# jiazhihao/ROC

Hardware: AMD Instinct MI355X
Metric: per-epoch training time (s), 2-layer GCN on Reddit (lower is better)
Workload: dtype bf16; 1 GPU; model=gcn-2layer-608-256-64, graph=reddit-synthetic-232965n-114848857e, global_batch=232965, parallelism=graph-partition x1 (single-gpu)

## Files before the change

### roc_amd/csrc/bindings.cpp

```cpp
#include <torch/extension.h>

void spmm(torch::Tensor out, torch::Tensor x, torch::Tensor rowptr,
          torch::Tensor colidx, c10::optional<torch::Tensor> deg_dst,
          c10::optional<torch::Tensor> deg_src,
          c10::optional<torch::Tensor> row_order, bool accumulate,
          int64_t col_base, int64_t ncols);
void rowscale(torch::Tensor out, torch::Tensor x, torch::Tensor scale);
void cast_rowscale(torch::Tensor out, torch::Tensor x,
                   c10::optional<torch::Tensor> scale);
void relu_fwd(torch::Tensor out, torch::Tensor x);
void sigmoid_fwd(torch::Tensor out, torch::Tensor x);
void relu_bwd(torch::Tensor dx, torch::Tensor dy, torch::Tensor y);
void sigmoid_bwd(torch::Tensor dx, torch::Tensor dy, torch::Tensor y);
void ewise_add(torch::Tensor out, torch::Tensor a, torch::Tensor b);
void ewise_mul(torch::Tensor out, torch::Tensor a, torch::Tensor b);
void dropout_fwd(torch::Tensor out, torch::Tensor x, double p, int64_t seed,
                 int64_t offset, c10::optional<torch::Tensor> counter);
void softmax_ce(torch::Tensor dl, torch::Tensor metrics, torch::Tensor logits,
                torch::Tensor labels, torch::Tensor mask, double grad_scale,
                int64_t num_classes);
void adam_step(torch::Tensor w, torch::Tensor g, torch::Tensor m,
               torch::Tensor v, double alpha, double b1, double b2, double eps,
               double wd, c10::optional<torch::Tensor> step,
               double decay_rate, int64_t decay_steps);
void gemm_rr(torch::Tensor C, torch::Tensor A, torch::Tensor Bt, bool relu,
             c10::optional<torch::Tensor> row_scale);
void gemm_atb(torch::Tensor C, torch::Tensor A, torch::Tensor B);
void spmm_refresh_knobs();
void spmm_edge(torch::Tensor out, torch::Tensor x, torch::Tensor rowptr,
               torch::Tensor colidx, torch::Tensor edge_val,
               c10::optional<torch::Tensor> deg_dst,
               c10::optional<torch::Tensor> row_order, bool accumulate);
void edge_dot(torch::Tensor dw, torch::Tensor dy, torch::Tensor x,
              torch::Tensor rowptr, torch::Tensor colidx);
void edge_softmax_fwd(torch::Tensor alpha, torch::Tensor s,
                      torch::Tensor rowptr);
void edge_softmax_bwd(torch::Tensor ds, torch::Tensor dalpha,
                      torch::Tensor alpha, torch::Tensor rowptr);
void att_softmax_fwd(torch::Tensor alpha, torch::Tensor s_src,
                     torch::Tensor s_dst, torch::Tensor rowptr,
                     torch::Tensor colidx, double slope);
void att_softmax_bwd(torch::Tensor dsrc, torch::Tensor dsdst,
                     torch::Tensor dalpha, torch::Tensor alpha,
                     torch::Tensor s_src, torch::Tensor s_dst,
                     torch::Tensor rowptr, torch::Tensor colidx,
                     double slope);
void register_graph_cpu(pybind11::module_& m);

PYBIND11_MODULE(TORCH_EXTENSION_NAME, m) {
  m.doc() = "roc_amd hand-written CDNA4 (gfx950) kernels";
  m.def("spmm", &spmm, "CSR SpMM neighbor aggregation (fused deg-norm)",
        pybind11::arg("out"), pybind11::arg("x"), pybind11::arg("rowptr"),
        pybind11::arg("colidx"), pybind11::arg("deg_dst") = pybind11::none(),
        pybind11::arg("deg_src") = pybind11::none(),
        pybind11::arg("row_order") = pybind11::none(),
        pybind11::arg("accumulate") = false,
        pybind11::arg("col_base") = 0, pybind11::arg("ncols") = 0);
  m.def("rowscale", &rowscale);
  m.def("cast_rowscale", &cast_rowscale,
        "fp32 -> bf16 cast with optional row scale (strip epilogue)",
        pybind11::arg("out"), pybind11::arg("x"),
        pybind11::arg("scale") = pybind11::none());
  m.def("relu_fwd", &relu_fwd);
  m.def("sigmoid_fwd", &sigmoid_fwd);
  m.def("relu_bwd", &relu_bwd);
  m.def("sigmoid_bwd", &sigmoid_bwd);
  m.def("ewise_add", &ewise_add);
  m.def("ewise_mul", &ewise_mul);
  m.def("dropout_fwd", &dropout_fwd, pybind11::arg("out"), pybind11::arg("x"),
        pybind11::arg("p"), pybind11::arg("seed"), pybind11::arg("offset"),
        pybind11::arg("counter") = pybind11::none());
  m.def("softmax_ce", &softmax_ce, pybind11::arg("dl"), pybind11::arg("metrics"),
        pybind11::arg("logits"), pybind11::arg("labels"), pybind11::arg("mask"),
        pybind11::arg("grad_scale"), pybind11::arg("num_classes") = -1);
  m.def("adam_step", &adam_step, pybind11::arg("w"), pybind11::arg("g"),
        pybind11::arg("m"), pybind11::arg("v"), pybind11::arg("alpha"),
        pybind11::arg("b1"), pybind11::arg("b2"), pybind11::arg("eps"),
        pybind11::arg("wd"), pybind11::arg("step") = pybind11::none(),
        pybind11::arg("decay_rate") = 1.0,
        pybind11::arg("decay_steps") = 100);
  m.def("gemm_rr", &gemm_rr, "C = A @ Bt^T (bf16 MFMA, fused relu/rowscale)",
        pybind11::arg("C"), pybind11::arg("A"), pybind11::arg("Bt"),
        pybind11::arg("relu"), pybind11::arg("row_scale") = pybind11::none());
  m.def("gemm_atb", &gemm_atb, "C += A^T @ B (fp32 split-K accumulate)");
  m.def("spmm_refresh_knobs", &spmm_refresh_knobs,
        "re-read ROC_SPMM_* env knobs (A/B harness only)");
  m.def("spmm_edge", &spmm_edge,
        "per-edge-weighted CSR SpMM (edge-tensor consumer)",
        pybind11::arg("out"), pybind11::arg("x"), pybind11::arg("rowptr"),
        pybind11::arg("colidx"), pybind11::arg("edge_val"),
        pybind11::arg("deg_dst") = pybind11::none(),
        pybind11::arg("row_order") = pybind11::none(),
        pybind11::arg("accumulate") = false);
  m.def("edge_dot", &edge_dot,
        "dw[e] = <dy[row_e], x[col_e]> (edge-value gradient)");
  m.def("edge_softmax_fwd", &edge_softmax_fwd,
        "per-row segment softmax over edge scores (GAT attention)");
  m.def("edge_softmax_bwd", &edge_softmax_bwd);
  m.def("att_softmax_fwd", &att_softmax_fwd,
        "fused GAT attention: lrelu(s_src[col]+s_dst[row]) -> softmax");
  m.def("att_softmax_bwd", &att_softmax_bwd);
  register_graph_cpu(m);
}
```

### roc_amd/csrc/spmm.hip

```cpp

#include "row_team.h"

namespace {

template <typename T>
struct RawVec { using type = float4; };
template <>
struct RawVec<unsigned short> { using type = uint4; };

__device__ __forceinline__ uint4 load_raw(const unsigned short* p) {
  return *reinterpret_cast<const uint4*>(p);
}
__device__ __forceinline__ float4 load_raw(const float* p) {
  return *reinterpret_cast<const float4*>(p);
}
__device__ __forceinline__ void acc_add(float* acc, const uint4& r, float w) {
  acc[0] += w * bf16_lo(r.x); acc[1] += w * bf16_hi(r.x);
  acc[2] += w * bf16_lo(r.y); acc[3] += w * bf16_hi(r.y);
  acc[4] += w * bf16_lo(r.z); acc[5] += w * bf16_hi(r.z);
  acc[6] += w * bf16_lo(r.w); acc[7] += w * bf16_hi(r.w);
}
__device__ __forceinline__ void acc_add(float* acc, const float4& r, float w) {
  acc[0] += w * r.x; acc[1] += w * r.y; acc[2] += w * r.z; acc[3] += w * r.w;
}

typedef __attribute__((ext_vector_type(4))) float f32x4v;

template <typename T>
struct GlobalGather {
  const T* x;
  int64_t D;
  int64_t col0;
  __device__ __forceinline__ typename RawVec<T>::type load(int u) const {
    return load_raw(x + (int64_t)u * D + col0);
  }
};

template <typename T>
struct BufferGather {
  __amdgpu_buffer_rsrc_t rsrc;
  unsigned dbytes;
  unsigned colbytes;
  __device__ __forceinline__ typename RawVec<T>::type load(int u) const {
    const f32x4v v = __builtin_amdgcn_raw_buffer_load_b128(
        rsrc, (unsigned)u * dbytes + colbytes, 0, 0);
    return __builtin_bit_cast(typename RawVec<T>::type, v);
  }
};

template <int N, typename T, typename LD, typename USE>
__device__ __forceinline__ void gather_group(
    const LD& ld, const int* __restrict__ colidx, int64_t e, USE&& use) {
  int u[N];
  typename RawVec<T>::type r[N];
#pragma unroll
  for (int i = 0; i < N; ++i) u[i] = colidx[e + i];
#pragma unroll
  for (int i = 0; i < N; ++i) r[i] = ld.load(u[i]);
#pragma unroll
  for (int i = 0; i < N; ++i) use(i, u[i], r[i]);
}

enum class Weight { kNone, kSrc, kEdge };

template <int N, typename T, Weight W, typename LD>
__device__ __forceinline__ void accum_group(
    float* __restrict__ acc, const LD& ld, const int* __restrict__ colidx,
    const float* __restrict__ weight, int64_t e) {
  float w[N];
  if constexpr (W == Weight::kEdge) {
#pragma unroll
    for (int i = 0; i < N; ++i) w[i] = weight[e + i];
  }
  gather_group<N, T>(ld, colidx, e,
                     [&](int i, int u, const typename RawVec<T>::type& r) {
    if constexpr (W == Weight::kEdge) acc_add(acc, r, w[i]);
    else if constexpr (W == Weight::kSrc) acc_add(acc, r, weight[u]);
    else acc_add(acc, r, 1.f);
  });
}

template <typename T, int UN, Weight W, typename LD>
__device__ __forceinline__ void row_accum_vec(
    float* __restrict__ acc, const LD& ld, const int* __restrict__ colidx,
    const float* __restrict__ weight, int64_t e, int64_t e1) {
  if constexpr (UN >= 16)
    for (; e + 15 < e1; e += 16) accum_group<16, T, W>(acc, ld, colidx, weight, e);
  if constexpr (UN >= 8)
    for (; e + 7 < e1; e += 8) accum_group<8, T, W>(acc, ld, colidx, weight, e);
  for (; e + 3 < e1; e += 4) accum_group<4, T, W>(acc, ld, colidx, weight, e);
  for (; e < e1; ++e) accum_group<1, T, W>(acc, ld, colidx, weight, e);
}

template <typename T, Weight W>
__device__ void row_accum_tail(
    float* __restrict__ acc, const T* __restrict__ x, int64_t ld, int64_t col0,
    int nvalid, const int* __restrict__ colidx,
    const float* __restrict__ weight, int64_t e0, int64_t e1) {
  for (int64_t e = e0; e < e1; ++e) {
    const int u0 = colidx[e];
    const T* r = x + (int64_t)u0 * ld + col0;
    const float w0 =
        W == Weight::kEdge ? weight[e] : (weight ? weight[u0] : 1.f);
    for (int j = 0; j < nvalid; ++j) acc[j] += w0 * elt_to_f32(r[j]);
  }
}

template <typename T, typename OT, int TEAM, int UN, bool BUF, Weight W>
__global__ __launch_bounds__(kBlock) void spmm_kernel(
    OT* __restrict__ out, const T* __restrict__ x,
    const int64_t* __restrict__ rowptr, const int* __restrict__ colidx,
    const float* __restrict__ deg_dst, const float* __restrict__ weight,
    const int* __restrict__ row_order, int num_rows, int64_t ld,
    int64_t col_base, int64_t col_end, bool accumulate, unsigned x_bytes) {
  constexpr int EPU = EltTraits<T>::kPerVec;
  const RowTeam<TEAM> rt;

  const int64_t col0 =
      col_base + ((int64_t)blockIdx.y * TEAM + rt.lane) * EPU;
  const bool full = (col0 + EPU) <= col_end;
  const int nvalid =
      full ? EPU : (col0 < col_end ? (int)(col_end - col0) : 0);

  if (full) {
    for (int ri = rt.team; ri < num_rows; ri += rt.nteams) {
      const int row = row_order ? row_order[ri] : ri;
      const int64_t e0 = rowptr[row];
      const int64_t e1 = rowptr[row + 1];
      float acc[EPU];
      OT* o = out + (int64_t)row * ld + col0;
      if (accumulate) {
#pragma unroll
        for (int j = 0; j < EPU; ++j) acc[j] = elt_to_f32(o[j]);
      } else {
#pragma unroll
        for (int j = 0; j < EPU; ++j) acc[j] = 0.f;
      }
      if constexpr (BUF) {
        BufferGather<T> g{
            __builtin_amdgcn_make_buffer_rsrc((void*)x, (short)0, x_bytes,
                                              0x00020000),
            (unsigned)(ld * sizeof(T)), (unsigned)(col0 * sizeof(T))};
        row_accum_vec<T, UN, W>(acc, g, colidx, weight, e0, e1);
      } else {
        GlobalGather<T> g{x, ld, col0};
        row_accum_vec<T, UN, W>(acc, g, colidx, weight, e0, e1);
      }
      if (deg_dst) {
        const float s = deg_dst[row];
#pragma unroll
        for (int j = 0; j < EPU; ++j) acc[j] *= s;
      }
      store_vec(o, acc);
    }
  } else if (nvalid > 0) {
    for (int ri = rt.team; ri < num_rows; ri += rt.nteams) {
      const int row = row_order ? row_order[ri] : ri;
      float acc[EPU];
      OT* o = out + (int64_t)row * ld + col0;
      for (int j = 0; j < nvalid; ++j)
        acc[j] = accumulate ? elt_to_f32(o[j]) : 0.f;
      row_accum_tail<T, W>(acc, x, ld, col0, nvalid, colidx, weight,
                           rowptr[row], rowptr[row + 1]);
      const float s = deg_dst ? deg_dst[row] : 1.f;
      for (int j = 0; j < nvalid; ++j) f32_to_elt(acc[j] * s, o + j);
    }
  }
}

struct SpmmKnobs {
  int team_override;
  int unroll;
  bool allow_buffer;
};

static SpmmKnobs read_spmm_knobs() {
  SpmmKnobs k{0, 16, true};
  if (const char* e = getenv("ROC_SPMM_TEAM")) {
    const int t = atoi(e);
    if (t == 8 || t == 16 || t == 32 || t == 64) k.team_override = t;
  }
  if (const char* e = getenv("ROC_SPMM_UNROLL")) k.unroll = atoi(e);
  if (const char* e = getenv("ROC_SPMM_BUFFER")) k.allow_buffer = e[0] != '0';
  return k;
}

static SpmmKnobs g_spmm_knobs;
static bool g_spmm_knobs_read = false;

static const SpmmKnobs& spmm_knobs() {
  if (!g_spmm_knobs_read) {
    g_spmm_knobs = read_spmm_knobs();
    g_spmm_knobs_read = true;
  }
  return g_spmm_knobs;
}

template <typename T, typename OT, int UN, Weight W>
void launch_spmm(OT* out, const T* x, const int64_t* rowptr,
                 const int* colidx, const float* deg_dst, const float* weight,
                 const int* row_order, int num_rows, int64_t ld,
                 int64_t col_base, int64_t col_end, bool accumulate,
                 size_t x_elems, int team_override, hipStream_t stream) {
  constexpr int EPU = EltTraits<T>::kPerVec;
  const int64_t units = (col_end - col_base + EPU - 1) / EPU;
  const int team = team_override ? team_override : row_team_size(units);
  const dim3 grid =
      row_team_grid(num_rows, team, (int)((units + team - 1) / team));
  const size_t xb = x_elems * sizeof(T);
  const bool buf = xb < (size_t)UINT_MAX && spmm_knobs().allow_buffer;
  const unsigned x_bytes = (unsigned)(buf ? xb : 0);
  if (team < 16) row_order = nullptr;
  dispatch_team(team, [&](auto team_c) {
    dispatch_bool(buf, [&](auto buf_c) {
      hipLaunchKernelGGL(
          (spmm_kernel<T, OT, decltype(team_c)::value, UN,
                       decltype(buf_c)::value, W>),
          grid, dim3(kBlock), 0, stream, out, x, rowptr, colidx, deg_dst,
          weight, row_order, num_rows, ld, col_base, col_end, accumulate,
          x_bytes);
    });
  });
}

template <typename T, int EPU>
__device__ __forceinline__ float dot_unit(
    const float (&a)[EPU], const typename RawVec<T>::type& r) {
  float b[EPU];
#pragma unroll
  for (int j = 0; j < EPU; ++j) b[j] = 0.f;
  acc_add(b, r, 1.f);
  float p = 0.f;
#pragma unroll
  for (int j = 0; j < EPU; ++j) p += a[j] * b[j];
  return p;
}

template <int N, typename T, int TEAM, int EPU>
__device__ __forceinline__ void edge_dot_group(
    float* __restrict__ dw, const float (&a)[EPU], const GlobalGather<T>& g,
    const int* __restrict__ colidx, int64_t e, bool live, int lane) {
  float p[N];
#pragma unroll
  for (int i = 0; i < N; ++i) p[i] = 0.f;
  if (live)
    gather_group<N, T>(g, colidx, e,
                       [&](int i, int, const typename RawVec<T>::type& r) {
      p[i] = dot_unit<T>(a, r);
    });
#pragma unroll
  for (int i = 0; i < N; ++i) p[i] = team_reduce_sum<TEAM>(p[i]);
  if (lane == 0) {
#pragma unroll
    for (int i = 0; i < N; ++i) dw[e + i] = p[i];
  }
}

template <typename T, int TEAM>
__global__ __launch_bounds__(kBlock) void edge_dot_kernel(
    float* __restrict__ dw, const T* __restrict__ dy,
    const T* __restrict__ x, const int64_t* __restrict__ rowptr,
    const int* __restrict__ colidx, int num_rows, int64_t D) {
  constexpr int EPU = EltTraits<T>::kPerVec;
  using Raw = typename RawVec<T>::type;
  const RowTeam<TEAM> rt;
  const int lane = rt.lane;
  if ((int64_t)TEAM * EPU >= D && D % EPU == 0) {
    const bool live = lane < (int)(D / EPU);
    const GlobalGather<T> g{x, D, (int64_t)lane * EPU};
    for (int row = rt.team; row < num_rows; row += rt.nteams) {
      const int64_t e0 = rowptr[row], e1 = rowptr[row + 1];
      float a[EPU] = {0.f};
      if (live) acc_add(a, load_raw(dy + (int64_t)row * D + g.col0), 1.f);
      int64_t e = e0;
      for (; e + 3 < e1; e += 4)
        edge_dot_group<4, T, TEAM>(dw, a, g, colidx, e, live, lane);
      for (; e < e1; ++e)
        edge_dot_group<1, T, TEAM>(dw, a, g, colidx, e, live, lane);
    }
    return;
  }
  for (int row = rt.team; row < num_rows; row += rt.nteams) {
    const int64_t e0 = rowptr[row], e1 = rowptr[row + 1];
    const T* dyr = dy + (int64_t)row * D;
    for (int64_t e = e0; e < e1; ++e) {
      const T* xr = x + (int64_t)colidx[e] * D;
      float p = 0.f;
      for (int64_t c = (int64_t)lane * EPU; c + EPU <= D;
           c += (int64_t)TEAM * EPU) {
        const Raw a = load_raw(dyr + c);
        const Raw b = load_raw(xr + c);
        float ta[EPU] = {0.f}, tb[EPU] = {0.f};
        acc_add(ta, a, 1.f);
        acc_add(tb, b, 1.f);
#pragma unroll
        for (int j = 0; j < EPU; ++j) p += ta[j] * tb[j];
      }
      for (int64_t j = (D / EPU) * EPU + lane; j < D; j += TEAM)
        p += elt_to_f32(dyr[j]) * elt_to_f32(xr[j]);
      p = team_reduce_sum<TEAM>(p);
      if (lane == 0) dw[e] = p;
    }
  }
}

template <typename T>
void launch_edge_dot(float* dw, const T* dy, const T* x,
                     const int64_t* rowptr, const int* colidx, int num_rows,
                     int64_t D, hipStream_t stream) {
  constexpr int EPU = EltTraits<T>::kPerVec;
  const int team = row_team_size((D + EPU - 1) / EPU);
  dispatch_team(team, [&](auto team_c) {
    hipLaunchKernelGGL((edge_dot_kernel<T, decltype(team_c)::value>),
                       row_team_grid(num_rows, team), dim3(kBlock), 0, stream,
                       dw, dy, x, rowptr, colidx, num_rows, D);
  });
}

void check_csr(const torch::Tensor& rowptr, const torch::Tensor& colidx,
               int num_rows) {
  ROC_CHECK_DEV_CONT(rowptr);
  ROC_CHECK_DEV_CONT(colidx);
  TORCH_CHECK(rowptr.scalar_type() == torch::kInt64, "rowptr must be int64");
  TORCH_CHECK(colidx.scalar_type() == torch::kInt32, "colidx must be int32");
  TORCH_CHECK(rowptr.size(0) == num_rows + 1, "rowptr size mismatch");
}

template <typename T>
const T* opt_ptr(const c10::optional<torch::Tensor>& t) {
  return t.has_value() ? t->data_ptr<T>() : nullptr;
}

}

void spmm_refresh_knobs() { g_spmm_knobs_read = false; }

void spmm(torch::Tensor out, torch::Tensor x, torch::Tensor rowptr,
          torch::Tensor colidx, c10::optional<torch::Tensor> deg_dst,
          c10::optional<torch::Tensor> deg_src,
          c10::optional<torch::Tensor> row_order, bool accumulate,
          int64_t col_base, int64_t ncols) {
  ROC_CHECK_DEV_CONT(out);
  ROC_CHECK_DEV_CONT(x);
  TORCH_CHECK(out.scalar_type() == x.scalar_type() ||
                  (out.scalar_type() == torch::kFloat32 &&
                   x.scalar_type() == torch::kBFloat16),
              "dtype mismatch (out must match x, or be fp32 for bf16 x)");
  const int num_rows = (int)out.size(0);
  const int64_t D = out.size(1);
  TORCH_CHECK(x.size(1) == D, "feature dim mismatch");
  check_csr(rowptr, colidx, num_rows);
  const int64_t col_end = ncols > 0 ? col_base + ncols : D;
  TORCH_CHECK(col_base >= 0 && col_base < col_end && col_end <= D,
              "bad column window");
  const float* ds = opt_ptr<float>(deg_src);
  const SpmmKnobs& kn = spmm_knobs();
  auto stream = roc_stream();
  dispatch_elt(x.scalar_type(), "spmm", [&](auto xt) {
    dispatch_elt(out.scalar_type(), "spmm", [&](auto ot) {
      using T = typename decltype(xt)::type;
      using OT = typename decltype(ot)::type;
      if constexpr (sizeof(OT) >= sizeof(T)) {
        auto go = [&](auto un_c, auto w_c) {
          launch_spmm<T, OT, decltype(un_c)::value, decltype(w_c)::value>(
              (OT*)out.data_ptr(), (const T*)x.data_ptr(),
              rowptr.data_ptr<int64_t>(), colidx.data_ptr<int>(),
              opt_ptr<float>(deg_dst), ds, opt_ptr<int>(row_order), num_rows,
              D, col_base, col_end, accumulate, (size_t)x.numel(),
              kn.team_override, stream);
        };
        auto by_weight = [&](auto un_c) {
          if (ds) go(un_c, std::integral_constant<Weight, Weight::kSrc>{});
          else go(un_c, std::integral_constant<Weight, Weight::kNone>{});
        };
        if (kn.unroll >= 16) by_weight(std::integral_constant<int, 16>{});
        else if (kn.unroll >= 8) by_weight(std::integral_constant<int, 8>{});
        else by_weight(std::integral_constant<int, 4>{});
      }
    });
  });
  ROC_HIP_CHECK(hipGetLastError());
}

void spmm_edge(torch::Tensor out, torch::Tensor x, torch::Tensor rowptr,
               torch::Tensor colidx, torch::Tensor edge_val,
               c10::optional<torch::Tensor> deg_dst,
               c10::optional<torch::Tensor> row_order, bool accumulate) {
  ROC_CHECK_DEV_CONT(out);
  ROC_CHECK_DEV_CONT(x);
  ROC_CHECK_DEV_CONT(edge_val);
  TORCH_CHECK(edge_val.scalar_type() == torch::kFloat32,
              "edge_val must be fp32");
  TORCH_CHECK(edge_val.numel() == colidx.numel(), "edge_val size mismatch");
  TORCH_CHECK(out.scalar_type() == x.scalar_type(), "dtype mismatch");
  const int num_rows = (int)out.size(0);
  const int64_t D = out.size(1);
  TORCH_CHECK(x.size(1) == D, "feature dim mismatch");
  check_csr(rowptr, colidx, num_rows);
  auto stream = roc_stream();
  dispatch_elt(x.scalar_type(), "spmm_edge", [&](auto xt) {
    using T = typename decltype(xt)::type;
    launch_spmm<T, T, 4, Weight::kEdge>(
        (T*)out.data_ptr(), (const T*)x.data_ptr(),
        rowptr.data_ptr<int64_t>(), colidx.data_ptr<int>(),
        opt_ptr<float>(deg_dst), edge_val.data_ptr<float>(),
        opt_ptr<int>(row_order), num_rows, D, 0, D, accumulate,
        (size_t)x.numel(), 0, stream);
  });
  ROC_HIP_CHECK(hipGetLastError());
}

void edge_dot(torch::Tensor dw, torch::Tensor dy, torch::Tensor x,
              torch::Tensor rowptr, torch::Tensor colidx) {
  ROC_CHECK_DEV_CONT(dw);
  ROC_CHECK_DEV_CONT(dy);
  ROC_CHECK_DEV_CONT(x);
  TORCH_CHECK(dw.scalar_type() == torch::kFloat32, "dw must be fp32");
  TORCH_CHECK(dw.numel() == colidx.numel(), "dw size mismatch");
  TORCH_CHECK(dy.scalar_type() == x.scalar_type(), "dtype mismatch");
  const int num_rows = (int)dy.size(0);
  const int64_t D = dy.size(1);
  TORCH_CHECK(x.size(1) == D, "feature dim mismatch");
  check_csr(rowptr, colidx, num_rows);
  auto stream = roc_stream();
  dispatch_elt(dy.scalar_type(), "edge_dot", [&](auto xt) {
    using T = typename decltype(xt)::type;
    launch_edge_dot<T>(dw.data_ptr<float>(), (const T*)dy.data_ptr(),
                       (const T*)x.data_ptr(), rowptr.data_ptr<int64_t>(),
                       colidx.data_ptr<int>(), num_rows, D, stream);
  });
  ROC_HIP_CHECK(hipGetLastError());
}
```

### roc_amd/ops/functional.py

```python
from __future__ import annotations

from typing import Optional

import torch

from . import reference as ref

try:
    from roc_amd import _C
except ImportError:
    _C = None


def has_ext() -> bool:
    return _C is not None


_PHASE_COLS: Optional[int] = None

_DW_STREAM = None
_DW_PENDING: list = []
_ASYNC_DW: Optional[bool] = None


def _async_dw() -> bool:
    global _ASYNC_DW
    if _ASYNC_DW is None:
        import os
        _ASYNC_DW = os.environ.get("ROC_ASYNC_DW", "0") == "1"
    return _ASYNC_DW


def _dw_stream():
    global _DW_STREAM
    if _DW_STREAM is None:
        _DW_STREAM = torch.cuda.Stream()
    return _DW_STREAM


def dw_flush() -> None:
    if not _DW_PENDING:
        return
    from .. import streamcheck
    cs = torch.cuda.current_stream()
    for done, _refs in _DW_PENDING:
        streamcheck.consumer(done, "dw-consume")
        cs.wait_event(done)
    _DW_PENDING.clear()


def _phase_cols() -> int:
    global _PHASE_COLS
    if _PHASE_COLS is None:
        import os
        _PHASE_COLS = int(os.environ.get("ROC_SPMM_PHASE_COLS", "0"))
    return _PHASE_COLS


def _hip(x: torch.Tensor) -> bool:
    if x.is_cuda:
        if _C is None:
            raise RuntimeError(
                "roc_amd._C extension is not built but a GPU tensor was passed. "
                "Run `python setup.py build_ext --inplace`. Refusing a silent "
                "eager fallback on GPU."
            )
        return True
    return False



def _strip_spmm(x, strips, num_rows, row_scale):
    D = x.shape[1]
    out32 = torch.empty(num_rows, D, dtype=torch.float32, device=x.device)
    ph = _phase_cols()
    if ph and D % ph == 0 and D // ph >= 2:
        phases = [(p, ph) for p in range(0, D, ph)]
    else:
        phases = [(0, 0)]
    for col_base, ncols in phases:
        for i, (srp, sci) in enumerate(strips):
            _C.spmm(out32, x, srp, sci, None, None, None, i > 0,
                    col_base, ncols)
    if x.dtype == torch.bfloat16 and D % 8 == 0:
        out = torch.empty(num_rows, D, dtype=torch.bfloat16, device=x.device)
        _C.cast_rowscale(out, out32, row_scale)
        return out
    if row_scale is not None:
        out32 = out32 * row_scale.unsqueeze(1)
    return out32.to(x.dtype)


class _SpMM(torch.autograd.Function):

    @staticmethod
    def forward(ctx, x, rowptr, colidx, t_rowptr, t_colidx, num_rows, num_ext,
                deg_dst, deg_src, row_order, t_row_order,
                fwd_strips=None, bwd_strips=None):
        ctx.save_for_backward(t_rowptr, t_colidx, deg_dst, deg_src, t_row_order)
        ctx.num_ext = num_ext
        ctx.bwd_strips = bwd_strips
        if _hip(x) and fwd_strips is not None and deg_src is None:
            out = _strip_spmm(x, fwd_strips, num_rows, deg_dst)
        elif _hip(x):
            out = torch.empty(num_rows, x.shape[1], dtype=x.dtype, device=x.device)
            _C.spmm(out, x, rowptr, colidx, deg_dst, deg_src, row_order)
        else:
            xin = x
            if deg_src is not None:
                xin = xin * deg_src.unsqueeze(1).to(xin.dtype)
            out = ref.spmm(xin, rowptr, colidx, num_rows)
            if deg_dst is not None:
                out = out * deg_dst.unsqueeze(1).to(out.dtype)
        return out

    @staticmethod
    def backward(ctx, dy):
        t_rowptr, t_colidx, deg_dst, deg_src, t_row_order = ctx.saved_tensors
        dy = dy.contiguous()
        if _hip(dy):
            if deg_dst is not None:
                tmp = torch.empty_like(dy)
                _C.rowscale(tmp, dy, deg_dst)
                dy = tmp
            if ctx.bwd_strips is not None and deg_src is None:
                dx = _strip_spmm(dy, ctx.bwd_strips, ctx.num_ext, None)
            else:
                dx = torch.empty(ctx.num_ext, dy.shape[1], dtype=dy.dtype,
                                 device=dy.device)
                _C.spmm(dx, dy, t_rowptr, t_colidx, deg_src, None, t_row_order)
        else:
            yin = dy
            if deg_dst is not None:
                yin = yin * deg_dst.unsqueeze(1).to(yin.dtype)
            dx = ref.spmm(yin, t_rowptr, t_colidx, ctx.num_ext)
            if deg_src is not None:
                dx = dx * deg_src.unsqueeze(1).to(dx.dtype)
        return (dx,) + (None,) * 12


class _SpMMEdge(torch.autograd.Function):

    @staticmethod
    def forward(ctx, x, w, rowptr, colidx, t_rowptr, t_colidx, t_eperm,
                num_rows, num_ext, dst_scale, row_order, t_row_order):
        w = w.contiguous()
        ctx.save_for_backward(x, w, rowptr, colidx, t_rowptr, t_colidx,
                              t_eperm, dst_scale, t_row_order)
        ctx.num_ext = num_ext
        if _hip(x):
            out = torch.empty(num_rows, x.shape[1], dtype=x.dtype,
                              device=x.device)
            _C.spmm_edge(out, x, rowptr, colidx, w, dst_scale, row_order,
                         False)
        else:
            out = ref.spmm_weighted(x, rowptr, colidx, w, num_rows)
            if dst_scale is not None:
                out = out * dst_scale.unsqueeze(1).to(out.dtype)
        return out

    @staticmethod
    def backward(ctx, dy):
        (x, w, rowptr, colidx, t_rowptr, t_colidx, t_eperm, dst_scale,
         t_row_order) = ctx.saved_tensors
        dy = dy.contiguous()
        need_x, need_w = ctx.needs_input_grad[0], ctx.needs_input_grad[1]
        dx = dw = None
        if _hip(dy):
            if dst_scale is not None:
                tmp = torch.empty_like(dy)
                _C.rowscale(tmp, dy, dst_scale)
                dy = tmp
            if need_x:
                t_w = w[t_eperm].contiguous()
                dx = torch.empty(ctx.num_ext, dy.shape[1], dtype=dy.dtype,
                                 device=dy.device)
                _C.spmm_edge(dx, dy, t_rowptr, t_colidx, t_w, None,
                             t_row_order, False)
            if need_w:
                dw = torch.empty_like(w)
                _C.edge_dot(dw, dy, x, rowptr, colidx)
        else:
            if dst_scale is not None:
                dy = dy * dst_scale.unsqueeze(1).to(dy.dtype)
            if need_x:
                dx = ref.spmm_weighted(dy, t_rowptr, t_colidx, w[t_eperm],
                                       ctx.num_ext)
            if need_w:
                dw = ref.edge_dot(dy, x, rowptr, colidx).to(w.dtype)
        return (dx, dw) + (None,) * 10


def scatter_gather_weighted(x, w, shard, dst_scale=None):
    return _SpMMEdge.apply(
        x, w, shard.rowptr, shard.colidx, shard.t_rowptr, shard.t_colidx,
        shard.t_edge_perm(), shard.n_local, shard.n_ext, dst_scale,
        shard.row_order, shard.t_row_order)


class _EdgeSoftmax(torch.autograd.Function):

    @staticmethod
    def forward(ctx, s, rowptr, row_of_edge):
        s = s.contiguous()
        if _hip(s):
            alpha = torch.empty_like(s)
            _C.edge_softmax_fwd(alpha, s, rowptr)
        else:
            n = rowptr.numel() - 1
            m = torch.full((n,), float("-inf"), dtype=s.dtype)
            m = m.scatter_reduce(0, row_of_edge, s, reduce="amax",
                                 include_self=True)
            ex = (s - m[row_of_edge]).exp()
            denom = torch.zeros(n, dtype=s.dtype).index_add_(
                0, row_of_edge, ex)
            alpha = ex / denom[row_of_edge]
        ctx.save_for_backward(alpha, rowptr, row_of_edge)
        return alpha

    @staticmethod
    def backward(ctx, dalpha):
        alpha, rowptr, row_of_edge = ctx.saved_tensors
        dalpha = dalpha.contiguous()
        if _hip(dalpha):
            ds = torch.empty_like(dalpha)
            _C.edge_softmax_bwd(ds, dalpha, alpha, rowptr)
        else:
            n = rowptr.numel() - 1
            dot = torch.zeros(n, dtype=alpha.dtype).index_add_(
                0, row_of_edge, alpha * dalpha)
            ds = alpha * (dalpha - dot[row_of_edge])
        return ds, None, None


def edge_softmax(scores, shard):
    return _EdgeSoftmax.apply(scores.float(), shard.rowptr,
                              shard.row_of_edge())


class _AttentionSoftmax(torch.autograd.Function):

    @staticmethod
    def forward(ctx, s_src, s_dst, rowptr, colidx, row_of_edge, slope):
        s_src = s_src.contiguous()
        s_dst = s_dst.contiguous()
        if _hip(s_src):
            alpha = torch.empty(colidx.numel(), dtype=torch.float32,
                                device=s_src.device)
            _C.att_softmax_fwd(alpha, s_src, s_dst, rowptr, colidx, slope)
        else:
            n = rowptr.numel() - 1
            sc = s_src[colidx.long()] + s_dst[row_of_edge]
            sc = torch.nn.functional.leaky_relu(sc, slope)
            m = torch.full((n,), float("-inf"), dtype=sc.dtype)
            m = m.scatter_reduce(0, row_of_edge, sc, reduce="amax",
                                 include_self=True)
            ex = (sc - m[row_of_edge]).exp()
            den = torch.zeros(n, dtype=sc.dtype).index_add_(
                0, row_of_edge, ex)
            alpha = ex / den[row_of_edge]
        ctx.save_for_backward(alpha, s_src, s_dst, rowptr, colidx,
                              row_of_edge)
        ctx.slope = slope
        return alpha

    @staticmethod
    def backward(ctx, dalpha):
        alpha, s_src, s_dst, rowptr, colidx, row_of_edge = ctx.saved_tensors
        slope = ctx.slope
        dalpha = dalpha.contiguous()
        if _hip(dalpha):
            dsrc = torch.zeros_like(s_src)
            dsdst = torch.empty_like(s_dst)
            _C.att_softmax_bwd(dsrc, dsdst, dalpha, alpha, s_src, s_dst,
                               rowptr, colidx, slope)
        else:
            n = rowptr.numel() - 1
            dot = torch.zeros(n, dtype=alpha.dtype).index_add_(
                0, row_of_edge, alpha * dalpha)
            ds = alpha * (dalpha - dot[row_of_edge])
            raw = s_src[colidx.long()] + s_dst[row_of_edge]
            dscore = torch.where(raw > 0, ds, slope * ds)
            dsrc = torch.zeros_like(s_src).index_add_(
                0, colidx.long(), dscore)
            dsdst = torch.zeros_like(s_dst).index_add_(
                0, row_of_edge, dscore)
        return dsrc, dsdst, None, None, None, None


def attention_softmax(s_src, s_dst, shard, slope: float = 0.2):
    return _AttentionSoftmax.apply(s_src.float(), s_dst.float(),
                                   shard.rowptr, shard.colidx,
                                   shard.row_of_edge(), slope)


def scatter_gather(x, shard, normalize: bool = False, dst_scale=None,
                   src_scale=None):
    deg_dst = shard.rsqrt_deg_local if normalize else dst_scale
    deg_src = shard.rsqrt_deg_ext if normalize else src_scale
    return _SpMM.apply(
        x, shard.rowptr, shard.colidx, shard.t_rowptr, shard.t_colidx,
        shard.n_local, shard.n_ext, deg_dst, deg_src,
        shard.row_order, shard.t_row_order,
        shard.fwd_strips, shard.bwd_strips,
    )



class _DegScale(torch.autograd.Function):

    @staticmethod
    def forward(ctx, x, scale):
        ctx.save_for_backward(scale)
        if _hip(x):
            out = torch.empty_like(x)
            _C.rowscale(out, x, scale)
        else:
            out = x * scale.unsqueeze(1).to(x.dtype)
        return out

    @staticmethod
    def backward(ctx, dy):
        (scale,) = ctx.saved_tensors
        dy = dy.contiguous()
        if _hip(dy):
            dx = torch.empty_like(dy)
            _C.rowscale(dx, dy, scale)
        else:
            dx = dy * scale.unsqueeze(1).to(dy.dtype)
        return dx, None


def indegree_norm(x, shard):
    return _DegScale.apply(x, shard.rsqrt_deg_local)


def degree_scale(x, scale):
    return _DegScale.apply(x, scale)



class _Linear(torch.autograd.Function):

    @staticmethod
    def forward(ctx, x, w, act, row_scale):
        if _hip(x):
            wt, wc = _cast_weight(w, x.dtype)
            ctx.wc = wc
            y = torch.empty(x.shape[0], w.shape[1], dtype=x.dtype, device=x.device)
            _C.gemm_rr(y, x, wt, act == "relu", row_scale)
            if act == "sigmoid":
                _C.sigmoid_fwd(y, y)
        else:
            y = ref.linear(x, w)
            if row_scale is not None:
                y = y * row_scale.unsqueeze(1).to(y.dtype)
            if act == "relu":
                y = ref.relu(y)
            elif act == "sigmoid":
                y = ref.sigmoid(y)
        ctx.save_for_backward(x, w, y if act else None, row_scale)
        ctx.act = act
        return y

    @staticmethod
    def backward(ctx, dy):
        x, w, y, row_scale = ctx.saved_tensors
        act = ctx.act
        dy = dy.contiguous()
        if _hip(dy):
            if act == "relu":
                dym = torch.empty_like(dy)
                _C.relu_bwd(dym, dy, y)
                dy = dym
            elif act == "sigmoid":
                dym = torch.empty_like(dy)
                _C.sigmoid_bwd(dym, dy, y)
                dy = dym
            if row_scale is not None:
                dym = torch.empty_like(dy)
                _C.rowscale(dym, dy, row_scale)
                dy = dym
            gbuf = w.grad if _async_dw() else None
            if (gbuf is not None and gbuf.dtype == torch.float32
                    and gbuf.is_contiguous() and gbuf.is_cuda):
                from .. import streamcheck
                s = _dw_stream()
# ... 254 lines not shown
```

### roc_amd/parallel/partition.py

```python
from __future__ import annotations

import os
from dataclasses import dataclass
from typing import List, Optional

import numpy as np
import torch

from ..graph import CSRGraph, build_transpose


def _gather_locality(rowptr: np.ndarray, colidx: np.ndarray,
                     max_sample: int = 1_000_000) -> float:
    ne = int(colidx.shape[0])
    if ne == 0:
        return 0.0
    if ne > max_sample:
        e = np.linspace(0, ne - 1, max_sample).astype(np.int64)
    else:
        e = np.arange(ne, dtype=np.int64)
    rows = np.searchsorted(rowptr, e, side="right") - 1
    return float((np.abs(rows - colidx[e].astype(np.int64)) < 8192).mean())


@dataclass
class GraphShard:

    rank: int
    world_size: int
    bounds: List[int]
    lo: int
    hi: int
    n_local: int
    n_halo: int
    n_ext: int
    rowptr: torch.Tensor
    colidx: torch.Tensor
    t_rowptr: torch.Tensor
    t_colidx: torch.Tensor
    deg_local: torch.Tensor
    rsqrt_deg_local: torch.Tensor
    inv_deg_local: torch.Tensor
    rsqrt_deg_ext: torch.Tensor
    row_order: Optional[torch.Tensor]
    t_row_order: Optional[torch.Tensor]
    halo_ids: torch.Tensor
    recv_splits: List[int]
    send_idx: torch.Tensor
    send_splits: List[int]
    loc_rowptr: Optional[torch.Tensor] = None
    loc_colidx: Optional[torch.Tensor] = None
    halo_rowptr: Optional[torch.Tensor] = None
    halo_colidx: Optional[torch.Tensor] = None
    t_loc_rowptr: Optional[torch.Tensor] = None
    t_loc_colidx: Optional[torch.Tensor] = None
    t_halo_rowptr: Optional[torch.Tensor] = None
    t_halo_colidx: Optional[torch.Tensor] = None
    comm_mode: str = "none"
    halo_fraction: float = 0.0
    ag_max_rows: int = 0
    ag_colidx: Optional[torch.Tensor] = None
    ag_t_rowptr: Optional[torch.Tensor] = None
    ag_t_colidx: Optional[torch.Tensor] = None
    ag_t_row_order: Optional[torch.Tensor] = None
    ag_self_rowptr: Optional[torch.Tensor] = None
    ag_self_colidx: Optional[torch.Tensor] = None
    ag_rem_rowptr: Optional[torch.Tensor] = None
    ag_rem_colidx: Optional[torch.Tensor] = None
    ag_self_row_order: Optional[torch.Tensor] = None
    ag_rem_row_order: Optional[torch.Tensor] = None
    ag_t_blk_order: Optional[torch.Tensor] = None
    fwd_strips: Optional[list] = None
    bwd_strips: Optional[list] = None

    def to(self, device) -> "GraphShard":
        d = {}
        for k, v in self.__dict__.items():
            if k.startswith("_"):
                continue
            if isinstance(v, torch.Tensor):
                v = v.to(device)
            elif isinstance(v, list) and v and isinstance(v[0], tuple):
                v = [tuple(t.to(device) for t in tup) for tup in v]
            d[k] = v
        return GraphShard(**d)

    @property
    def has_overlap_split(self) -> bool:
        return self.loc_rowptr is not None

    @property
    def num_local_edges(self) -> int:
        return int(self.colidx.numel())

    def colidx_long(self) -> torch.Tensor:
        c = getattr(self, "_colidx_long", None)
        if c is None:
            c = self.colidx.long()
            object.__setattr__(self, "_colidx_long", c)
        return c

    def row_of_edge(self) -> torch.Tensor:
        r = getattr(self, "_row_of_edge", None)
        if r is None:
            deg = (self.rowptr[1:] - self.rowptr[:-1]).long()
            r = torch.repeat_interleave(
                torch.arange(self.n_local, dtype=torch.long,
                             device=self.rowptr.device), deg)
            object.__setattr__(self, "_row_of_edge", r)
        return r

    def t_edge_perm(self) -> torch.Tensor:
        p = getattr(self, "_t_eperm", None)
        if p is None:
            p = torch.argsort(self.colidx.long(), stable=True)
            object.__setattr__(self, "_t_eperm", p)
        return p


def build_strip_plan(rowptr: torch.Tensor, colidx: torch.Tensor,
                     num_cols: int, width: int):
    rp = rowptr.numpy()
    ci = colidx.numpy()
    nrows = rp.shape[0] - 1
    ci64 = ci.astype(np.int64)
    row = np.repeat(np.arange(nrows, dtype=np.int64), np.diff(rp))
    key = row * (num_cols + 1) + ci64
    rows_q = np.arange(nrows, dtype=np.int64) * (num_cols + 1)
    pos = [rp[:-1].astype(np.int64)]
    for b in range(width, num_cols, width):
        pos.append(np.searchsorted(key, rows_q + b))
    pos.append(rp[1:].astype(np.int64))
    strips = []
    for s in range(len(pos) - 1):
        seg_start, seg_end = pos[s], pos[s + 1]
        cnt = seg_end - seg_start
        srp = np.zeros(nrows + 1, dtype=np.int64)
        np.cumsum(cnt, out=srp[1:])
        if srp[-1]:
            idx = np.repeat(seg_start - srp[:-1], cnt) + np.arange(
                int(srp[-1]), dtype=np.int64)
            sci = np.ascontiguousarray(ci[idx])
        else:
            sci = np.empty(0, dtype=ci.dtype)
        strips.append((torch.from_numpy(srp), torch.from_numpy(sci)))
    return strips


def edge_tensor(shard: GraphShard, dim: Optional[int] = None,
                dtype=torch.float32, init: str = "zeros") -> torch.Tensor:
    e = shard.num_local_edges
    dev = shard.colidx.device
    shape = (e,) if dim is None else (e, dim)
    if init == "zeros":
        return torch.zeros(*shape, dtype=dtype, device=dev)
    if init == "ones":
        return torch.ones(*shape, dtype=dtype, device=dev)
    if init == "gcn_norm":
        assert dim is None, "gcn_norm is a scalar-per-edge init"
        deg = (shard.rowptr[1:] - shard.rowptr[:-1])
        row_of_edge = torch.repeat_interleave(
            torch.arange(shard.n_local, dtype=torch.long, device=dev), deg)
        val = (shard.rsqrt_deg_local[row_of_edge]
               * shard.rsqrt_deg_ext[shard.colidx.long()])
        return val.to(dtype)
    raise ValueError(f"unknown edge_tensor init {init!r}")


def edge_balanced_bounds(rowptr: torch.Tensor, num_parts: int) -> List[int]:
    rp = rowptr.numpy()
    e = int(rp[-1])
    n = rp.shape[0] - 1
    targets = [(e * k) // num_parts for k in range(num_parts + 1)]
    bounds = np.searchsorted(rp, targets, side="left").tolist()
    bounds[0], bounds[-1] = 0, n
    for i in range(1, len(bounds)):
        bounds[i] = max(bounds[i], bounds[i - 1])
    return bounds


def fit_cost_model(samples: List[tuple]) -> tuple:
    A = np.array([[s[0], s[1]] for s in samples], dtype=np.float64)
    y = np.array([s[2] for s in samples], dtype=np.float64)
    a = float((A[:, 0] * y).sum() / max((A[:, 0] ** 2).sum(), 1e-30))
    b = 0.0
    if len(samples) >= 3 and np.linalg.matrix_rank(A) == 2:
        coef, *_ = np.linalg.lstsq(A, y, rcond=None)
        if coef[0] > 0 and coef[1] >= 0:
            a, b = float(coef[0]), float(coef[1])
    return a, b


def rebalance_bounds_comm(rowptr: torch.Tensor, bounds: List[int],
                          per_rank_time: List[float],
                          per_rank_halo: List[int],
                          samples: Optional[List[tuple]] = None) -> List[int]:
    rp = rowptr.numpy().astype(np.float64)
    p = len(bounds) - 1
    edges = [rp[bounds[k + 1]] - rp[bounds[k]] for k in range(p)]
    cur = [(edges[k], float(per_rank_halo[k]), per_rank_time[k])
           for k in range(p)]
    if samples is not None:
        samples.extend(cur)
        cur = samples[-8 * p:]
    a, b = fit_cost_model(cur)
    T = sum(per_rank_time) / p
    e_total = rp[-1]
    floor = 0.05 * e_total / p
    budget = [max((T - b * per_rank_halo[k]) / max(a, 1e-30), floor)
              for k in range(p)]
    scale = e_total / sum(budget)
    targets = np.cumsum([0.0] + [bk * scale for bk in budget])
    nb = np.searchsorted(rp, targets, side="left").tolist()
    nb[0], nb[-1] = 0, rowptr.numel() - 1
    for i in range(1, len(nb)):
        nb[i] = max(nb[i], nb[i - 1])
    return nb


def rebalance_bounds(rowptr: torch.Tensor, bounds: List[int],
                     per_rank_time: List[float]) -> List[int]:
    rp = rowptr.numpy().astype(np.float64)
    p = len(bounds) - 1
    edges = [rp[bounds[k + 1]] - rp[bounds[k]] for k in range(p)]
    thr = [edges[k] / max(per_rank_time[k], 1e-9) for k in range(p)]
    total_thr = sum(thr)
    e_total = rp[-1]
    targets = np.cumsum([0.0] + [e_total * t / total_thr for t in thr])
    nb = np.searchsorted(rp, targets, side="left").tolist()
# ... 125 lines not shown
        t_row_order = None
    else:
        row_order = np.argsort(-local_deg_edges, kind="stable").astype(np.int32)
        t_deg = np.diff(t_rowptr.numpy())
        t_row_order = np.argsort(-t_deg, kind="stable").astype(np.int32)

    shard_kw = {}
    if world_size > 1:
        shard_kw["comm_mode"] = comm_mode
        shard_kw["halo_fraction"] = float(halo_fraction)
    if world_size > 1 and comm_mode == "allgather":
        sizes = [bounds[r + 1] - bounds[r] for r in range(world_size)]
        mr = max(sizes)
        owners = np.searchsorted(bounds, local_cols_global,
                                 side="right") - 1
        ag_cols = (owners.astype(np.int64) * mr +
                   (local_cols_global - np.asarray(bounds)[owners]))
        shard_kw["ag_max_rows"] = int(mr)
        shard_kw["ag_colidx"] = torch.from_numpy(ag_cols.astype(np.int32))
        ag_t = build_transpose(world_size * mr, rowptr_t,
                               shard_kw["ag_colidx"])
        shard_kw["ag_t_rowptr"], shard_kw["ag_t_colidx"] = ag_t
        ag_t_deg = np.diff(ag_t[0].numpy())
        shard_kw["ag_t_row_order"] = torch.from_numpy(
            np.argsort(-ag_t_deg, kind="stable").astype(np.int32))
        is_self = owners == rank
        row_of_edge = np.repeat(np.arange(n_local, dtype=np.int64),
                                np.diff(local_rowptr))
        for key_pfx, sel, cols in (
                ("ag_self", is_self,
                 (local_cols_global - lo).astype(np.int32)),
                ("ag_rem", ~is_self, ag_cols.astype(np.int32))):
            rows_sel = row_of_edge[sel]
            cnt = np.bincount(rows_sel, minlength=n_local).astype(np.int64)
            part_rp = np.zeros(n_local + 1, dtype=np.int64)
            np.cumsum(cnt, out=part_rp[1:])
            shard_kw[f"{key_pfx}_rowptr"] = torch.from_numpy(part_rp)
            shard_kw[f"{key_pfx}_colidx"] = torch.from_numpy(
                np.ascontiguousarray(cols[sel]))
            shard_kw[f"{key_pfx}_row_order"] = torch.from_numpy(
                np.argsort(-cnt, kind="stable").astype(np.int32))
        ag_t_rp = ag_t[0].numpy()
        blk_ord = np.empty(world_size * mr, dtype=np.int32)
        for r in range(world_size):
            deg_blk = np.diff(ag_t_rp[r * mr:(r + 1) * mr + 1])
            blk_ord[r * mr:(r + 1) * mr] = np.argsort(
                -deg_blk, kind="stable").astype(np.int32)
        shard_kw["ag_t_blk_order"] = torch.from_numpy(blk_ord)
    if world_size > 1 and comm_mode == "halo":
        is_loc_edge = colidx < n_local
        row_of_edge = np.repeat(np.arange(n_local, dtype=np.int64),
                                np.diff(local_rowptr))
        for key_pfx, sel in (("loc", is_loc_edge), ("halo", ~is_loc_edge)):
            rows_sel = row_of_edge[sel]
            cols_sel = colidx[sel].astype(np.int32)
            if key_pfx == "halo":
                cols_sel = cols_sel - n_local
            cnt = np.bincount(rows_sel, minlength=n_local).astype(np.int64)
            part_rp = np.zeros(n_local + 1, dtype=np.int64)
            np.cumsum(cnt, out=part_rp[1:])
            shard_kw[f"{key_pfx}_rowptr"] = torch.from_numpy(part_rp)
            shard_kw[f"{key_pfx}_colidx"] = torch.from_numpy(
                np.ascontiguousarray(cols_sel))
        t_loc = build_transpose(n_local, shard_kw["loc_rowptr"],
                                shard_kw["loc_colidx"])
        t_halo = build_transpose(max(n_halo, 0), shard_kw["halo_rowptr"],
                                 shard_kw["halo_colidx"])
        shard_kw["t_loc_rowptr"], shard_kw["t_loc_colidx"] = t_loc
        shard_kw["t_halo_rowptr"], shard_kw["t_halo_colidx"] = t_halo

    phase_on = int(os.environ.get("ROC_SPMM_PHASE_COLS", "0")) > 0
    strip_w = int(os.environ.get("ROC_SPMM_STRIP_WIDTH",
                                 "65536" if phase_on else "16384"))
    strip_min = int(os.environ.get("ROC_SPMM_STRIP_MIN_EDGES",
                                   str(24_000_000)))
    max_k = int(os.environ.get("ROC_SPMM_STRIP_MAX_K", "32"))
    n_strips = (n_ext + strip_w - 1) // max(strip_w, 1)
    if (strip_w > 0 and colidx_t.numel() >= strip_min
            and 2 <= n_strips <= max_k):
        shard_kw["fwd_strips"] = build_strip_plan(rowptr_t, colidx_t,
                                                  n_ext, strip_w)
        shard_kw["bwd_strips"] = build_strip_plan(t_rowptr, t_colidx,
                                                  n_local, strip_w)

    return GraphShard(
        rank=rank, world_size=world_size, bounds=list(bounds),
        lo=lo, hi=hi, n_local=n_local, n_halo=n_halo, n_ext=n_ext,
        rowptr=rowptr_t, colidx=colidx_t,
        t_rowptr=t_rowptr, t_colidx=t_colidx, **shard_kw,
        deg_local=torch.from_numpy(deg_local.copy()),
        rsqrt_deg_local=torch.from_numpy(1.0 / np.sqrt(deg_local)),
        inv_deg_local=torch.from_numpy(1.0 / deg_local),
        rsqrt_deg_ext=torch.from_numpy(1.0 / np.sqrt(deg_ext)),
        row_order=(torch.from_numpy(row_order)
                   if row_order is not None else None),
        t_row_order=(torch.from_numpy(t_row_order)
                     if t_row_order is not None else None),
        halo_ids=torch.from_numpy(halo_ids),
        recv_splits=recv_splits,
        send_idx=send_idx,
        send_splits=send_splits,
    )
```

Measured before the change: 0.01586 s/epoch.

## Schedule heavy rows first in strip SpMM and fuse final bf16 cast

```diff
diff --git a/roc_amd/csrc/bindings.cpp b/roc_amd/csrc/bindings.cpp
--- a/roc_amd/csrc/bindings.cpp
+++ b/roc_amd/csrc/bindings.cpp
@@ -4,7 +4,9 @@
           torch::Tensor colidx, c10::optional<torch::Tensor> deg_dst,
           c10::optional<torch::Tensor> deg_src,
           c10::optional<torch::Tensor> row_order, bool accumulate,
-          int64_t col_base, int64_t ncols);
+          int64_t col_base, int64_t ncols,
+          c10::optional<torch::Tensor> heavy_rows, int64_t heavy_min,
+          c10::optional<torch::Tensor> final_out);
 void rowscale(torch::Tensor out, torch::Tensor x, torch::Tensor scale);
 void cast_rowscale(torch::Tensor out, torch::Tensor x,
                    c10::optional<torch::Tensor> scale);
@@ -55,7 +57,10 @@
         pybind11::arg("deg_src") = pybind11::none(),
         pybind11::arg("row_order") = pybind11::none(),
         pybind11::arg("accumulate") = false,
-        pybind11::arg("col_base") = 0, pybind11::arg("ncols") = 0);
+        pybind11::arg("col_base") = 0, pybind11::arg("ncols") = 0,
+        pybind11::arg("heavy_rows") = pybind11::none(),
+        pybind11::arg("heavy_min") = 0,
+        pybind11::arg("final_out") = pybind11::none());
   m.def("rowscale", &rowscale);
   m.def("cast_rowscale", &cast_rowscale,
         "fp32 -> bf16 cast with optional row scale (strip epilogue)",
diff --git a/roc_amd/csrc/spmm.hip b/roc_amd/csrc/spmm.hip
--- a/roc_amd/csrc/spmm.hip
+++ b/roc_amd/csrc/spmm.hip
@@ -106,13 +106,16 @@
   }
 }
 
-template <typename T, typename OT, int TEAM, int UN, bool BUF, Weight W>
+template <typename T, typename OT, int TEAM, int UN, bool BUF, Weight W,
+          bool HEAVY = false, bool FINAL = false>
 __global__ __launch_bounds__(kBlock) void spmm_kernel(
     OT* __restrict__ out, const T* __restrict__ x,
     const int64_t* __restrict__ rowptr, const int* __restrict__ colidx,
     const float* __restrict__ deg_dst, const float* __restrict__ weight,
     const int* __restrict__ row_order, int num_rows, int64_t ld,
-    int64_t col_base, int64_t col_end, bool accumulate, unsigned x_bytes) {
+    int64_t col_base, int64_t col_end, bool accumulate, unsigned x_bytes,
+    const int* __restrict__ heavy_rows, int num_heavy, int heavy_min,
+    unsigned short* __restrict__ final_out) {
   constexpr int EPU = EltTraits<T>::kPerVec;
   const RowTeam<TEAM> rt;
 
@@ -123,10 +126,7 @@
       full ? EPU : (col0 < col_end ? (int)(col_end - col0) : 0);
 
   if (full) {
-    for (int ri = rt.team; ri < num_rows; ri += rt.nteams) {
-      const int row = row_order ? row_order[ri] : ri;
-      const int64_t e0 = rowptr[row];
-      const int64_t e1 = rowptr[row + 1];
+    auto do_row = [&](int row, int64_t e0, int64_t e1) {
       float acc[EPU];
       OT* o = out + (int64_t)row * ld + col0;
       if (accumulate) {
@@ -151,7 +151,36 @@
 #pragma unroll
         for (int j = 0; j < EPU; ++j) acc[j] *= s;
       }
-      store_vec(o, acc);
+      if constexpr (FINAL) store_vec(final_out + (int64_t)row * ld + col0, acc);
+      else store_vec(o, acc);
+    };
+    if constexpr (HEAVY) {
+      constexpr int TPW = 64 / TEAM;
+      const int lt = (int)threadIdx.x / TEAM;
+      int h = ((lt / TPW) * (int)gridDim.x + (int)blockIdx.x) * TPW + lt % TPW;
+      int ri = rt.team;
+      for (;;) {
+        int row;
+        const bool from_list = h < num_heavy;
+        if (from_list) {
+          row = heavy_rows[h];
+          h += rt.nteams;
+          if ((unsigned)row >= (unsigned)num_rows) continue;
+        } else {
+          if (ri >= num_rows) break;
+          row = ri;
+          ri += rt.nteams;
+        }
+        const int64_t e0 = rowptr[row];
+        const int64_t e1 = rowptr[row + 1];
+        if (!from_list && e1 - e0 >= heavy_min) continue;
+        do_row(row, e0, e1);
+      }
+    } else {
+      for (int ri = rt.team; ri < num_rows; ri += rt.nteams) {
+        const int row = row_order ? row_order[ri] : ri;
+        do_row(row, rowptr[row], rowptr[row + 1]);
+      }
     }
   } else if (nvalid > 0) {
     for (int ri = rt.team; ri < num_rows; ri += rt.nteams) {
@@ -163,7 +192,12 @@
       row_accum_tail<T, W>(acc, x, ld, col0, nvalid, colidx, weight,
                            rowptr[row], rowptr[row + 1]);
       const float s = deg_dst ? deg_dst[row] : 1.f;
-      for (int j = 0; j < nvalid; ++j) f32_to_elt(acc[j] * s, o + j);
+      if constexpr (FINAL) {
+        unsigned short* fo = final_out + (int64_t)row * ld + col0;
+        for (int j = 0; j < nvalid; ++j) f32_to_elt(acc[j] * s, fo + j);
+      } else {
+        for (int j = 0; j < nvalid; ++j) f32_to_elt(acc[j] * s, o + j);
+      }
     }
   }
 }
@@ -196,12 +230,22 @@
   return g_spmm_knobs;
 }
 
-template <typename T, typename OT, int UN, Weight W>
+struct StripPass {
+  bool heavy = false;
+  const int* heavy_rows = nullptr;
+  int num_heavy = 0;
+  int heavy_min = 0;
+  unsigned short* final_out = nullptr;
+};
+
+template <typename T, typename OT, int UN, Weight W, bool HEAVY = false,
+          bool FINAL = false>
 void launch_spmm(OT* out, const T* x, const int64_t* rowptr,
                  const int* colidx, const float* deg_dst, const float* weight,
                  const int* row_order, int num_rows, int64_t ld,
                  int64_t col_base, int64_t col_end, bool accumulate,
-                 size_t x_elems, int team_override, hipStream_t stream) {
+                 size_t x_elems, int team_override, hipStream_t stream,
+                 const StripPass& sp = {}) {
   constexpr int EPU = EltTraits<T>::kPerVec;
   const int64_t units = (col_end - col_base + EPU - 1) / EPU;
   const int team = team_override ? team_override : row_team_size(units);
@@ -215,10 +259,10 @@
     dispatch_bool(buf, [&](auto buf_c) {
       hipLaunchKernelGGL(
           (spmm_kernel<T, OT, decltype(team_c)::value, UN,
-                       decltype(buf_c)::value, W>),
+                       decltype(buf_c)::value, W, HEAVY, FINAL>),
           grid, dim3(kBlock), 0, stream, out, x, rowptr, colidx, deg_dst,
           weight, row_order, num_rows, ld, col_base, col_end, accumulate,
-          x_bytes);
+          x_bytes, sp.heavy_rows, sp.num_heavy, sp.heavy_min, sp.final_out);
     });
   });
 }
@@ -339,9 +383,41 @@
           torch::Tensor colidx, c10::optional<torch::Tensor> deg_dst,
           c10::optional<torch::Tensor> deg_src,
           c10::optional<torch::Tensor> row_order, bool accumulate,
-          int64_t col_base, int64_t ncols) {
+          int64_t col_base, int64_t ncols,
+          c10::optional<torch::Tensor> heavy_rows, int64_t heavy_min,
+          c10::optional<torch::Tensor> final_out) {
   ROC_CHECK_DEV_CONT(out);
   ROC_CHECK_DEV_CONT(x);
+  StripPass sp;
+  if (heavy_rows.has_value() || final_out.has_value()) {
+    TORCH_CHECK(out.scalar_type() == torch::kFloat32 &&
+                    x.scalar_type() == torch::kBFloat16 &&
+                    !deg_src.has_value(),
+                "heavy_rows / final_out are strip-pass options: bf16 x, "
+                "fp32 out, no deg_src");
+  }
+  if (heavy_rows.has_value()) {
+    ROC_CHECK_DEV_CONT(*heavy_rows);
+    TORCH_CHECK(heavy_rows->scalar_type() == torch::kInt32,
+                "heavy_rows must be int32");
+    TORCH_CHECK(!row_order.has_value(),
+                "heavy_rows and row_order are exclusive");
+    TORCH_CHECK(heavy_min >= 0 && heavy_min <= INT_MAX, "bad heavy_min");
+    sp.heavy = true;
+    sp.heavy_rows = heavy_rows->data_ptr<int>();
+    sp.num_heavy = (int)heavy_rows->numel();
+    sp.heavy_min = (int)heavy_min;
+  }
+  if (final_out.has_value()) {
+    ROC_CHECK_DEV_CONT(*final_out);
+    TORCH_CHECK(final_out->scalar_type() == torch::kBFloat16,
+                "final_out must be bf16");
+    TORCH_CHECK(final_out->sizes() == out.sizes(),
+                "final_out shape mismatch");
+    TORCH_CHECK(col_base == 0 && ncols == 0,
+                "final_out needs a whole-row pass");
+    sp.final_out = (unsigned short*)final_out->data_ptr();
+  }
   TORCH_CHECK(out.scalar_type() == x.scalar_type() ||
                   (out.scalar_type() == torch::kFloat32 &&
                    x.scalar_type() == torch::kBFloat16),
@@ -362,12 +438,28 @@
       using OT = typename decltype(ot)::type;
       if constexpr (sizeof(OT) >= sizeof(T)) {
         auto go = [&](auto un_c, auto w_c) {
-          launch_spmm<T, OT, decltype(un_c)::value, decltype(w_c)::value>(
-              (OT*)out.data_ptr(), (const T*)x.data_ptr(),
-              rowptr.data_ptr<int64_t>(), colidx.data_ptr<int>(),
-              opt_ptr<float>(deg_dst), ds, opt_ptr<int>(row_order), num_rows,
-              D, col_base, col_end, accumulate, (size_t)x.numel(),
-              kn.team_override, stream);
+          constexpr int UN = decltype(un_c)::value;
+          constexpr Weight W = decltype(w_c)::value;
+          auto launch = [&](auto heavy_c, auto final_c) {
+            launch_spmm<T, OT, UN, W, decltype(heavy_c)::value,
+                        decltype(final_c)::value>(
+                (OT*)out.data_ptr(), (const T*)x.data_ptr(),
+                rowptr.data_ptr<int64_t>(), colidx.data_ptr<int>(),
+                opt_ptr<float>(deg_dst), ds, opt_ptr<int>(row_order),
+                num_rows, D, col_base, col_end, accumulate,
+                (size_t)x.numel(), kn.team_override, stream, sp);
+          };
+          if constexpr (std::is_same_v<T, unsigned short> &&
+                        std::is_same_v<OT, float> && W == Weight::kNone) {
+            if (sp.heavy || sp.final_out) {
+              dispatch_bool(sp.heavy, [&](auto heavy_c) {
+                dispatch_bool(sp.final_out != nullptr,
+                              [&](auto final_c) { launch(heavy_c, final_c); });
+              });
+              return;
+            }
+          }
+          launch(std::false_type{}, std::false_type{});
         };
         auto by_weight = [&](auto un_c) {
           if (ds) go(un_c, std::integral_constant<Weight, Weight::kSrc>{});
diff --git a/roc_amd/ops/functional.py b/roc_amd/ops/functional.py
--- a/roc_amd/ops/functional.py
+++ b/roc_amd/ops/functional.py
@@ -70,7 +70,7 @@
 
 
 
-def _strip_spmm(x, strips, num_rows, row_scale):
+def _strip_spmm(x, strips, num_rows, row_scale, heavy=None, heavy_min=0):
     D = x.shape[1]
     out32 = torch.empty(num_rows, D, dtype=torch.float32, device=x.device)
     ph = _phase_cols()
@@ -78,10 +78,24 @@
         phases = [(p, ph) for p in range(0, D, ph)]
     else:
         phases = [(0, 0)]
+    bf16 = x.dtype == torch.bfloat16
+    fuse_final = bf16 and D % 8 == 0 and phases == [(0, 0)]
+    if not bf16:
+        heavy = None
+    out = None
     for col_base, ncols in phases:
         for i, (srp, sci) in enumerate(strips):
-            _C.spmm(out32, x, srp, sci, None, None, None, i > 0,
-                    col_base, ncols)
+            hv = heavy[i] if heavy is not None else None
+            if fuse_final and i == len(strips) - 1:
+                out = torch.empty(num_rows, D, dtype=torch.bfloat16,
+                                  device=x.device)
+                _C.spmm(out32, x, srp, sci, row_scale, None, None, i > 0,
+                        0, 0, hv, heavy_min, out)
+            else:
+                _C.spmm(out32, x, srp, sci, None, None, None, i > 0,
+                        col_base, ncols, hv, heavy_min)
+    if out is not None:
+        return out
     if x.dtype == torch.bfloat16 and D % 8 == 0:
         out = torch.empty(num_rows, D, dtype=torch.bfloat16, device=x.device)
         _C.cast_rowscale(out, out32, row_scale)
@@ -96,12 +110,15 @@
     @staticmethod
     def forward(ctx, x, rowptr, colidx, t_rowptr, t_colidx, num_rows, num_ext,
                 deg_dst, deg_src, row_order, t_row_order,
-                fwd_strips=None, bwd_strips=None):
+                fwd_strips=None, bwd_strips=None, fwd_heavy=None,
+                bwd_heavy=None, heavy_min=0):
         ctx.save_for_backward(t_rowptr, t_colidx, deg_dst, deg_src, t_row_order)
         ctx.num_ext = num_ext
         ctx.bwd_strips = bwd_strips
+        ctx.bwd_heavy = (bwd_heavy, heavy_min)
         if _hip(x) and fwd_strips is not None and deg_src is None:
-            out = _strip_spmm(x, fwd_strips, num_rows, deg_dst)
+            out = _strip_spmm(x, fwd_strips, num_rows, deg_dst, fwd_heavy,
+                              heavy_min)
         elif _hip(x):
             out = torch.empty(num_rows, x.shape[1], dtype=x.dtype, device=x.device)
             _C.spmm(out, x, rowptr, colidx, deg_dst, deg_src, row_order)
@@ -124,7 +141,8 @@
                 _C.rowscale(tmp, dy, deg_dst)
                 dy = tmp
             if ctx.bwd_strips is not None and deg_src is None:
-                dx = _strip_spmm(dy, ctx.bwd_strips, ctx.num_ext, None)
+                dx = _strip_spmm(dy, ctx.bwd_strips, ctx.num_ext, None,
+                                 *ctx.bwd_heavy)
             else:
                 dx = torch.empty(ctx.num_ext, dy.shape[1], dtype=dy.dtype,
                                  device=dy.device)
@@ -136,7 +154,7 @@
             dx = ref.spmm(yin, t_rowptr, t_colidx, ctx.num_ext)
             if deg_src is not None:
                 dx = dx * deg_src.unsqueeze(1).to(dx.dtype)
-        return (dx,) + (None,) * 12
+        return (dx,) + (None,) * 15
 
 
 class _SpMMEdge(torch.autograd.Function):
@@ -303,6 +321,9 @@
         shard.n_local, shard.n_ext, deg_dst, deg_src,
         shard.row_order, shard.t_row_order,
         shard.fwd_strips, shard.bwd_strips,
+        getattr(shard, "fwd_strip_heavy", None),
+        getattr(shard, "bwd_strip_heavy", None),
+        getattr(shard, "strip_heavy_min", 0),
     )
 
 
diff --git a/roc_amd/parallel/partition.py b/roc_amd/parallel/partition.py
--- a/roc_amd/parallel/partition.py
+++ b/roc_amd/parallel/partition.py
@@ -72,6 +72,9 @@
     ag_t_blk_order: Optional[torch.Tensor] = None
     fwd_strips: Optional[list] = None
     bwd_strips: Optional[list] = None
+    fwd_strip_heavy: Optional[list] = None
+    bwd_strip_heavy: Optional[list] = None
+    strip_heavy_min: int = 0
 
     def to(self, device) -> "GraphShard":
         d = {}
@@ -82,6 +85,8 @@
                 v = v.to(device)
             elif isinstance(v, list) and v and isinstance(v[0], tuple):
                 v = [tuple(t.to(device) for t in tup) for tup in v]
+            elif isinstance(v, list) and v and isinstance(v[0], torch.Tensor):
+                v = [t.to(device) for t in v]
             d[k] = v
         return GraphShard(**d)
 
@@ -145,6 +150,28 @@
             sci = np.empty(0, dtype=ci.dtype)
         strips.append((torch.from_numpy(srp), torch.from_numpy(sci)))
     return strips
+
+
+HEAVY_MIN_DEFAULT = 128
+_HEAVY_MIN: Optional[int] = None
+
+
+def strip_heavy_min() -> int:
+    global _HEAVY_MIN
+    if _HEAVY_MIN is None:
+        _HEAVY_MIN = max(0, int(os.environ.get("ROC_SPMM_HEAVY_MIN",
+                                               str(HEAVY_MIN_DEFAULT))))
+    return _HEAVY_MIN
+
+
+def build_strip_heavy(strips, heavy_min: int):
+    heavy = []
+    for srp, _ in strips:
+        seg = np.diff(srp.numpy())
+        rows = np.nonzero(seg >= heavy_min)[0]
+        rows = rows[np.argsort(-seg[rows], kind="stable")]
+        heavy.append(torch.from_numpy(rows.astype(np.int32)))
+    return heavy
 
 
 def edge_tensor(shard: GraphShard, dim: Optional[int] = None,
@@ -436,6 +463,13 @@
                                                   n_ext, strip_w)
         shard_kw["bwd_strips"] = build_strip_plan(t_rowptr, t_colidx,
                                                   n_local, strip_w)
+        heavy_min = strip_heavy_min()
+        if heavy_min > 0:
+            shard_kw["fwd_strip_heavy"] = build_strip_heavy(
+                shard_kw["fwd_strips"], heavy_min)
+            shard_kw["bwd_strip_heavy"] = build_strip_heavy(
+                shard_kw["bwd_strips"], heavy_min)
+            shard_kw["strip_heavy_min"] = heavy_min
 
     return GraphShard(
         rank=rank, world_size=world_size, bounds=list(bounds),
```

Result: faster. 0.01434 s/epoch, median of 6 (-9.6%).
